# triq-org/spectroplot-js

Hardware: AMD Instinct MI355X
Metric: STFT frames/sec (N=1024 cf32) + IQ MSamples/s end-to-end to RGBA (higher is better)
Workload: dtype f64; 1 GPU; 16 MSample cf32, N=1024, Blackman-Harris, Viridis, gain 6, range 30, spectrogram layout, 16384 frames per GPU; format=CF32, n=1024, samples_per_gpu=16777216, frames_per_gpu=16384, window=blackmanHarris, cmap=viridis, generator=trinoise seed=0x5EED0001 step=7321 gshift=11 amp=0.5 namp=0.02

## Files before the change

### spectroplot-js_amd/binding.py

```python
import ctypes as C
import os
import weakref
import subprocess

import numpy as np

_HERE = os.path.dirname(os.path.abspath(__file__))

SP_CB_HIST_SIZE = 1000
FORMATS = ["CU4", "CS4", "CU8", "CS8", "CU12", "CS12", "CU16", "CS16", "CU32", "CS32", "CU64", "CS64", "CF32", "CF64"]

SP_ERR_NOT_POW2 = -2
SP_ERR_BYTE_LENGTH = -3
SP_ERR_UNSUPPORTED = -4
SP_ERR_NO_DEVICE = -5
SP_ERR_INVALID_ARG = -1

DETECTORS = {"sample": 0, "peak": 1}


def detector_id(detector):
    if detector not in DETECTORS:
        raise SpectroplotError(SP_ERR_INVALID_ARG, "detector must be 'sample' or 'peak', not %r" % (detector,))
    return DETECTORS[detector]
# ... 518 lines not shown

    def set_mean_window(self, nbytes=0):
        self._chk(self.lib.L.sp_context_set_mean_window(self.h, int(nbytes)))

    def render_index(self, fmt, data, n, windowc, block_norm, gain, rng, lut, width, channel_mode=False, waterfall=False,
                     detector="sample", want_index=True, fill=None):
        fid, _ = parse_format(fmt)
        data = np.ascontiguousarray(data, dtype=np.uint8)
        req, keep = _make_request(fid, n, windowc, block_norm, gain, rng, lut, channel_mode, waterfall, detector)
        W = int(width)
        L = len(keep[1])
        out, mm, rep = _host_reply(W, n, L, "index", 1, fill)
        self._chk(self.lib.L.sp_render_index(self.h, C.byref(req), _p(data), data.size, W, C.byref(rep),
                                             _p(out["index"]) if want_index else None))
        out["dBfs_min"], out["dBfs_max"] = float(mm[0]), float(mm[1])
        return out

    def index_to_rgba(self, d_index, pixels, lut, d_rgba):
        lut = np.ascontiguousarray(lut, dtype=np.uint8).reshape(-1, 3)
        self._chk(self.lib.L.sp_index_to_rgba(self.h, C.c_void_p(d_index or None), int(pixels), lut.ctypes.data_as(C.c_void_p), len(lut),
                                              C.c_void_p(d_rgba or None)))

    def render_density(self, fmt, data, n, windowc, block_norm, gain, rng, lut, width, channel_mode=False, waterfall=False,
                       detector="sample", fill=None):
        fid, _ = parse_format(fmt)
        data = np.ascontiguousarray(data, dtype=np.uint8)
        req, keep = _make_request(fid, n, windowc, block_norm, gain, rng, lut, channel_mode, waterfall, detector)
        out = np.full((int(n), len(keep[1])), 0 if fill is None else int(fill), np.uint32)
        self._chk(self.lib.L.sp_render_density(self.h, C.byref(req), data.ctypes.data_as(C.c_void_p), data.size, int(width),
                                               out.ctypes.data_as(C.c_void_p)))
        return out

    def density_from_index(self, d_index, n, width, waterfall, lut_len, d_density, accumulate=False):
        self._chk(self.lib.L.sp_density_from_index(self.h, C.c_void_p(d_index or None), int(n), int(width), int(bool(waterfall)),
                                                   int(lut_len), C.c_void_p(d_density or None), int(bool(accumulate))))

    def plan_creations(self):
        n = C.c_int64()
        self._chk(self.lib.L.sp_context_plan_creations(self.h, C.byref(n)))
        return n.value

    def plan(self, fmt, n, windowc, block_norm, gain, rng, lut, channel_mode=False, waterfall=False, detector="sample"):
        return Plan(self, fmt, n, windowc, block_norm, gain, rng, lut, channel_mode, waterfall, detector)


class Plan:

    def __init__(self, ctx, fmt, n, windowc, block_norm, gain, rng, lut, channel_mode=False, waterfall=False, detector="sample"):
        self.ctx = ctx
        self.detector = detector
        self.n = int(n)
        self.fid, self.sample_width = parse_format(fmt)
        req, keep = _make_request(self.fid, n, windowc, block_norm, gain, rng, lut, channel_mode, waterfall, detector)
        self.lut_len = len(keep[1])
        h = C.c_void_p()
        ctx._chk(ctx.lib.L.sp_plan_create(ctx.h, C.byref(req), C.byref(h)))
        self.h = h
        ctx._plans.add(self)

    def close(self):
        if self.h:
            self.ctx.lib.L.sp_plan_destroy(self.h)
            self.h = None

    def __del__(self):
        try:
            self.close()
        except Exception:
            pass

    def kernel_name(self, nbytes=None, width=None):
        if nbytes is None:
            return self.ctx.lib.L.sp_plan_kernel_name(self.h).decode()
        return self.ctx.lib.L.sp_plan_kernel_name_for(self.h, int(nbytes), int(width)).decode()

    def debug_launch(self, nbytes, width, rgba=0):
        out = np.zeros(len(LAUNCH_FIELDS), np.int64)
        used = C.c_size_t()
        self.ctx._chk(self.ctx.lib.L.sp_plan_debug_launch(self.h, int(nbytes), int(width), C.c_void_p(rgba or None),
                                                          out.ctypes.data_as(C.c_void_p), len(out), C.byref(used)))
        return _launch_dict(out)

    def force_kernel(self, which):
        self.ctx._chk(self.ctx.lib.L.sp_plan_force_kernel(self.h, {"auto": 0, "scratch": 1, "frames": 3}[which]))

    def execute(self, d_bytes, nbytes, width, rgba=0, gauge_mins=0, gauge_maxs=0, gauge_amps=0, c_hist=0, cb_hist=0, dbfs_minmax=0):
        rep = _device_reply(rgba, gauge_mins, gauge_maxs, gauge_amps, c_hist, cb_hist, dbfs_minmax)
        self.ctx._chk(self.ctx.lib.L.sp_plan_execute(self.h, C.c_void_p(d_bytes), nbytes, int(width), C.byref(rep)))

    def traces_kernel_name_for(self, nbytes, width):
        return self.ctx.lib.L.sp_plan_traces_kernel_name_for(self.h, int(nbytes), int(width)).decode()

    def execute_traces(self, d_bytes, nbytes, width, trace_min=0, trace_max=0):
        self.ctx._chk(self.ctx.lib.L.sp_plan_execute_traces(self.h, C.c_void_p(d_bytes or None), int(nbytes), int(width),
                                                            C.c_void_p(trace_min or None), C.c_void_p(trace_max or None)))

    def power_kernel_name_for(self, nbytes, width):
        return self.ctx.lib.L.sp_plan_power_kernel_name_for(self.h, int(nbytes), int(width)).decode()

    def execute_power(self, d_bytes, nbytes, width, d_power):
        self.ctx._chk(self.ctx.lib.L.sp_plan_execute_power(self.h, C.c_void_p(d_bytes or None), int(nbytes), int(width),
                                                           C.c_void_p(d_power or None)))

    def mean_kernel_name_for(self, nbytes, width):
        return self.ctx.lib.L.sp_plan_mean_kernel_name_for(self.h, int(nbytes), int(width)).decode()

    def execute_mean(self, d_bytes, nbytes, width, d_mean):
        self.ctx._chk(self.ctx.lib.L.sp_plan_execute_mean(self.h, C.c_void_p(d_bytes or None), int(nbytes), int(width),
                                                          C.c_void_p(d_mean or None)))

    def bandpower_kernel_name_for(self, nbytes, width):
        return self.ctx.lib.L.sp_plan_bandpower_kernel_name_for(self.h, int(nbytes), int(width)).decode()

    def execute_bandpower(self, d_bytes, nbytes, width, bands, d_band):
        b, count = _band_array(bands)
        self.ctx._chk(self.ctx.lib.L.sp_plan_execute_bandpower(self.h, C.c_void_p(d_bytes or None), int(nbytes), int(width),
                                                               _p(b) if count else None, count, C.c_void_p(d_band or None)))

    def power_to_db(self, d_power, count, d_db):
        self.ctx._chk(self.ctx.lib.L.sp_plan_power_to_db(self.h, C.c_void_p(d_power or None), int(count), C.c_void_p(d_db or None)))

    def index_kernel_name_for(self, nbytes, width):
        return self.ctx.lib.L.sp_plan_index_kernel_name_for(self.h, int(nbytes), int(width)).decode()

    def debug_index_launch(self, nbytes, width, index=0):
        out = np.zeros(len(LAUNCH_FIELDS), np.int64)
        used = C.c_size_t()
        self.ctx._chk(self.ctx.lib.L.sp_plan_debug_index_launch(self.h, int(nbytes), int(width), C.c_void_p(index or None),
                                                                out.ctypes.data_as(C.c_void_p), len(out), C.byref(used)))
        return _launch_dict(out)

    def execute_index(self, d_bytes, nbytes, width, index=0, rgba=0, gauge_mins=0, gauge_maxs=0, gauge_amps=0, c_hist=0, cb_hist=0,
                      dbfs_minmax=0):
        rep = _device_reply(rgba, gauge_mins, gauge_maxs, gauge_amps, c_hist, cb_hist, dbfs_minmax)
        self.ctx._chk(self.ctx.lib.L.sp_plan_execute_index(self.h, C.c_void_p(d_bytes or None), int(nbytes), int(width), C.byref(rep),
                                                           C.c_void_p(index or None)))

    def execute_density(self, d_bytes, nbytes, width, d_density, accumulate=False):
        self.ctx._chk(self.ctx.lib.L.sp_plan_execute_density(self.h, C.c_void_p(d_bytes or None), int(nbytes), int(width),
                                                             C.c_void_p(d_density or None), int(bool(accumulate))))

    def execute_batch(self, items):
        arr = (_BatchItem * max(len(items), 1))()
        keys = ("rgba", "gauge_mins", "gauge_maxs", "gauge_amps", "c_hist", "cb_hist", "dbfs_minmax")
        for k, (d_bytes, nbytes, width, outs) in enumerate(items):
            arr[k].bytes = d_bytes or None
            arr[k].nbytes = int(nbytes)
            arr[k].width = int(width)
            arr[k].reply = _device_reply(*[outs.get(key) for key in keys])
        self.ctx._chk(self.ctx.lib.L.sp_plan_execute_batch(self.h, arr, len(items)))

    def execute_from_host(self, data, width, rgba=0, gauge_mins=0, gauge_maxs=0, gauge_amps=0, c_hist=0, cb_hist=0, dbfs_minmax=0):
        data = np.ascontiguousarray(data, dtype=np.uint8)
        rep = _device_reply(rgba, gauge_mins, gauge_maxs, gauge_amps, c_hist, cb_hist, dbfs_minmax)
        self.ctx._chk(self.ctx.lib.L.sp_plan_execute_from_host(self.h, data.ctypes.data_as(C.c_void_p), data.size, int(width), C.byref(rep)))
        return data


class Group:

    def __init__(self, devices):
        self.lib = Library.get()
        arr = (C.c_int32 * len(devices))(*devices)
        h = C.c_void_p()
        self.lib.check(self.lib.L.sp_group_create(arr, len(devices), C.byref(h)))
        self.h = h
        self.size = len(devices)
# ... 52 lines not shown
```

### spectroplot-js_amd/csrc/sp_api.hip

```cpp
#include <hip/hip_runtime.h>

#include <cmath>
#include <cstdio>
#include <cstdlib>
#include <cstring>
#include <new>
#include <string>
#include <vector>

#include "../../include/spectroplot_hip.h"
#include "sp_geometry.h"
#include "sp_host.h"
#include "sp_kernel_frames_batch.h"
#include "sp_kernel_frames_peak.h"
#include "sp_kernel_frames_traces.h"
#include "sp_kernel_frames_power.h"
#include "sp_kernel_frames_index.h"
#include "sp_launch.h"
#include "sp_exact_sum.h"
#include "sp_cmap_tables.h"

namespace {

struct DeviceBuffer {
    void *p = nullptr;
    size_t cap = 0;
    int reserve(size_t bytes)
    {
        if (bytes <= cap) return SP_OK;
        if (p) (void)hipFree(p);
        p = nullptr;
        cap = 0;
        size_t want = bytes + bytes / 8 + 256;
        if (hipMalloc(&p, want) != hipSuccess) {
            if (hipMalloc(&p, bytes) != hipSuccess) return SP_ERR_NOMEM;
            want = bytes;
        }
        cap = want;
        return SP_OK;
    }
    void release()
    {
        if (p) (void)hipFree(p);
        p = nullptr;
        cap = 0;
    }
};

struct HostBuffer {
    void *p = nullptr;
    size_t cap = 0;
    int reserve(size_t bytes)
    {
        if (bytes <= cap) return SP_OK;
        if (p) (void)hipHostFree(p);
        p = nullptr;
        cap = 0;
        const size_t want = bytes + bytes / 8 + 256;
        if (hipHostMalloc(&p, want, hipHostMallocDefault) != hipSuccess) return SP_ERR_NOMEM;
        cap = want;
        return SP_OK;
    }
    void release()
    {
        if (p) (void)hipHostFree(p);
        p = nullptr;
        cap = 0;
    }
};

struct NamedRequest {
    std::string format, window, cmap;
    int32_t n = 0, channel_mode = 0, waterfall = 0;
    double gain = 0, range = 0;
    std::vector<double> windowc;
    std::vector<uint8_t> lut;
    double block_norm = 0;
    static std::string str(const char *s) { return s ? s : ""; }
    bool same(const sp_named_request &r) const
    {
        return !windowc.empty() && format == str(r.format) && window == str(r.window) && cmap == str(r.cmap) && n == r.n
               && channel_mode == (r.channel_mode ? 1 : 0) && waterfall == (r.waterfall ? 1 : 0) && !memcmp(&gain, &r.gain, 8)
               && !memcmp(&range, &r.range, 8);
    }
};

}

struct sp_context {
    int device = 0;
    hipStream_t own_stream = nullptr;
    hipStream_t stream = nullptr;
    std::string error;
    int cu_count = 256;
    DeviceBuffer frame_minmax;
    DeviceBuffer partial;
    DeviceBuffer scratch;
    DeviceBuffer traces_ws;
    DeviceBuffer power_plane;
    DeviceBuffer mean_ws;
    DeviceBuffer mean_window;
    size_t mean_window_bytes = 0;
    DeviceBuffer index_rgba;
    DeviceBuffer density_index;
    DeviceBuffer density_reply;
    DeviceBuffer in_bytes, out_rgba, render_small;
    HostBuffer host_small;
    hipStream_t copy_in = nullptr, copy_out = nullptr;
    hipEvent_t ev_arrived[spgeo::kMaxChunks] = {}, ev_rendered[spgeo::kMaxChunks] = {};
    sp_plan *cached_plan = nullptr;
    NamedRequest named;
    long long plans_created = 0;
    bool acc_dirty = false;
    size_t last_upload_bytes = 0;
    int last_chunks = 0;
    uint32_t seq = 0;
    DeviceBuffer batch_dev;
    HostBuffer batch_host;
    hipEvent_t ev_batch = nullptr;
    hipEvent_t ev_batch_done = nullptr;
    bool timing = false;
    hipEvent_t ev0 = nullptr, ev1 = nullptr;
    bool timed = false;
};

enum Kernel {
    kKernelAuto = 0,
    kKernelScratch = 1,
    kKernelLdsR16 = 2,
    kKernelFrames = 3,
    kKernelFramesPeak = 4,
};
static bool finishes_request(int kernel) { return kernel == kKernelFrames || kernel == kKernelFramesPeak; }

struct sp_plan {
    sp_context *ctx = nullptr;
    sp_request req{};
    std::vector<double> window;
    std::vector<uint8_t> lut;
    int levels = 0;
    spfmt::Format fmt{};
    double block_norm_db = 0;
    float gray_a = 0, gray_b = 0, cb_a = 0, cb_b = 0;
    bool edges_in_f32 = false;
    bool taper_finite = false;
    bool tw16_ok = false;
    sphost::Thresholds th{};
    DeviceBuffer tables;
    const double *d_window = nullptr, *d_cos = nullptr, *d_sin = nullptr, *d_gray_edge = nullptr, *d_cb_edge = nullptr;
    const uint32_t *d_lut = nullptr;
    const uint16_t *d_cell_g = nullptr, *d_cell_l = nullptr;
    const double2 *d_stage_tw = nullptr;
    DeviceBuffer ident_lut;
    int force_kernel = kKernelAuto;
};

namespace {

int fail(sp_context *ctx, int code, const std::string &msg)
{
    if (ctx) ctx->error = msg;
    return code;
}

int hip_fail(sp_context *ctx, hipError_t e, const char *what)
{
    return fail(ctx, SP_ERR_HIP, std::string(what) + ": " + hipGetErrorString(e));
}

#define SP_HIP(ctx, call)                                            \
    do {                                                             \
        hipError_t e_ = (call);                                      \
        if (e_ != hipSuccess) return hip_fail((ctx), e_, #call);     \
    } while (0)

int validate_request(sp_context *ctx, const sp_request *r)
{
    std::string why;
    const int rc = sphost::validate_request(r, why);
    return rc ? fail(ctx, rc, why) : SP_OK;
}

template <typename Body>
int timed(sp_context *ctx, Body &&body)
{
    if (ctx->timing) SP_HIP(ctx, hipEventRecord(ctx->ev0, ctx->stream));
    const int rc = body();
    if (rc) return rc;
    if (ctx->timing) {
        SP_HIP(ctx, hipEventRecord(ctx->ev1, ctx->stream));
        ctx->timed = true;
    }
    return SP_OK;
}

}


extern "C" int sp_version(void) { return SP_VERSION; }

extern "C" const char *sp_status_string(int status)
{
    switch (status) {
    case SP_OK: return "ok";
    case SP_ERR_INVALID_ARG: return "invalid argument";
    case SP_ERR_NOT_POW2: return "Length is not a power of 2";
    case SP_ERR_BYTE_LENGTH: return "byte length is not a multiple of the element size";
    case SP_ERR_UNSUPPORTED: return "unsupported by this library";
    case SP_ERR_NO_DEVICE: return "no HIP device";
    case SP_ERR_HIP: return "HIP runtime error";
    case SP_ERR_NOMEM: return "out of device memory";
    default: return "unknown status";
    }
}

extern "C" const char *sp_last_error(const sp_context *ctx) { return ctx ? ctx->error.c_str() : ""; }

extern "C" int sp_format_parse(const char *name, int32_t *format, int32_t *sample_width)
{
    const int32_t id = sphost::parse_format(name ? name : "");
    if (format) *format = id;
    if (sample_width) *sample_width = spfmt::describe(id).width;
    return SP_OK;
}

extern "C" int sp_format_element_size(int32_t format)
{
    if (format < 0 || format >= SP_FMT_COUNT) return SP_ERR_INVALID_ARG;
    return spfmt::describe(format).elem;
}

extern "C" int sp_slice_bounds(size_t nbytes, int32_t sample_width, int32_t index, int32_t count, size_t *begin, size_t *end)
{
    if (sample_width < 1 || count < 1 || index < 0 || index >= count || !begin || !end) return SP_ERR_INVALID_ARG;
    const size_t end_sample = nbytes / (size_t)sample_width;
// ... 243 lines not shown

extern "C" int sp_device_memset(sp_context *ctx, void *d_ptr, int value, size_t nbytes)
{
    if (!ctx) return SP_ERR_INVALID_ARG;
    SP_HIP(ctx, hipSetDevice(ctx->device));
    SP_HIP(ctx, hipMemsetAsync(d_ptr, value, nbytes, ctx->stream));
    return SP_OK;
}

extern "C" int sp_synth_trinoise(sp_context *ctx, void *d_bytes, int32_t format, uint64_t t0, uint64_t count, uint32_t seed,
                                 uint32_t step, uint32_t gshift, double amp, double namp)
{
    if (!ctx || !d_bytes) return SP_ERR_INVALID_ARG;
    if (format < 0 || format >= SP_FMT_COUNT) return fail(ctx, SP_ERR_INVALID_ARG, "unknown format id");
    if (count == 0) return SP_OK;
    SP_HIP(ctx, hipSetDevice(ctx->device));
    const spk::SynthArgs a{(uint8_t *)d_bytes, t0, count, seed, step, gshift, amp, namp};
    const int rc = spk::launch_synth_trinoise(a, format, ctx->stream);
    if (rc) return rc == SP_ERR_UNSUPPORTED ? fail(ctx, rc, "synth: too many samples for one launch") : rc;
    SP_HIP(ctx, hipGetLastError());
    return SP_OK;
}


extern "C" int sp_plan_create(sp_context *ctx, const sp_request *req, sp_plan **out)
{
    if (!ctx || !out) return SP_ERR_INVALID_ARG;
    *out = nullptr;
    int rc = validate_request(ctx, req);
    if (rc) return rc;
    SP_HIP(ctx, hipSetDevice(ctx->device));

    sp_plan *p = new (std::nothrow) sp_plan;
    if (!p) return fail(ctx, SP_ERR_NOMEM, "out of host memory");
    p->ctx = ctx;
    p->req = *req;
    p->window.assign(req->windowc, req->windowc + req->n);
    p->lut.assign(req->lut_rgb, req->lut_rgb + 3 * (size_t)req->lut_len);
    p->req.windowc = nullptr;
    p->req.lut_rgb = nullptr;
    p->levels = sphost::log2_exact(req->n);
    p->fmt = spfmt::describe(req->format);

    const int n = req->n, half = n / 2, L = req->lut_len;
    std::vector<double> ct((size_t)half), st((size_t)half);
    sphost::twiddles(n, ct.data(), st.data());
    const sphost::PixelMath pm(req->block_norm, req->gain, req->range, L);
    const sphost::Thresholds th = sphost::build_thresholds(pm, L);
    p->block_norm_db = pm.block_norm_db;
    p->gray_a = th.gray_a;
    p->gray_b = th.gray_b;
    p->cb_a = th.cb_a;
    p->cb_b = th.cb_b;
    p->edges_in_f32 = true;
    for (int g = 1; g < L; g++) p->edges_in_f32 &= th.gray_edge[(size_t)g] >= 0x1p-100 && th.gray_edge[(size_t)g] <= 0x1p100;
    for (int j = 1; j <= SP_CB_HIST_SIZE; j++) p->edges_in_f32 &= th.cb_edge[(size_t)j] >= 0x1p-100 && th.cb_edge[(size_t)j] <= 0x1p100;
    p->taper_finite = true;
    for (int i = 0; i < n; i++) p->taper_finite &= std::isfinite(p->window[(size_t)i]);
    p->tw16_ok = n >= 16;
    for (int k = 0; k < 8 && p->tw16_ok; k++)
        p->tw16_ok = ct[(size_t)k * (size_t)(n / 16)] == spk2::kTw16Host[k].c && st[(size_t)k * (size_t)(n / 16)] == spk2::kTw16Host[k].s;
    p->th = th;
    p->th.gray_edge.clear();
    p->th.cb_edge.clear();
    p->th.cell_g.clear();
    p->th.cell_l.clear();
    std::vector<uint32_t> lut32((size_t)L);
    for (int i = 0; i < L; i++)
        lut32[(size_t)i] = (uint32_t)p->lut[3 * (size_t)i] | ((uint32_t)p->lut[3 * (size_t)i + 1] << 8)
                           | ((uint32_t)p->lut[3 * (size_t)i + 2] << 16) | 0xff000000u;
    std::vector<double2> stage_tw;
    if (spk::frame_parts_support(n)) {
        stage_tw.resize((size_t)n);
        stage_tw[0] = make_double2(0, 0);
        for (int s = 1; s <= p->levels; s++) {
            const int cnt = 1 << (s - 1);
            for (int m = 0; m < cnt; m++) {
                const int k = m << (p->levels - s);
                stage_tw[(size_t)(cnt + m)] = make_double2(ct[(size_t)k], st[(size_t)k]);
            }
        }
    }

    const size_t nd = (size_t)n + 2 * (size_t)half + (size_t)L + (SP_CB_HIST_SIZE + 1) + 2 * stage_tw.size();
    const size_t cell_u16 = th.cell_g.size() + th.cell_l.size();
    const size_t bytes = nd * sizeof(double) + (((size_t)L * sizeof(uint32_t) + 7) & ~(size_t)7) + cell_u16 * sizeof(uint16_t);
    rc = p->tables.reserve(bytes);
    if (rc) {
        delete p;
        return fail(ctx, rc, "plan tables: out of device memory");
    }
    std::vector<uint8_t> host(bytes);
    double *h = (double *)host.data();
    double *d = (double *)p->tables.p;
    size_t o = 0;
    auto put = [&](const void *src, size_t count) {
        if (count) memcpy(h + o, src, count * sizeof(double));
        const double *dev = d + o;
        o += count;
        return dev;
    };
    p->d_window = put(p->window.data(), (size_t)n);
    p->d_cos = put(ct.data(), (size_t)half);
    p->d_sin = put(st.data(), (size_t)half);
    p->d_gray_edge = put(th.gray_edge.data(), (size_t)L);
    p->d_cb_edge = put(th.cb_edge.data(), SP_CB_HIST_SIZE + 1);
    p->d_stage_tw = (const double2 *)put(stage_tw.data(), 2 * stage_tw.size());
    memcpy(h + o, lut32.data(), (size_t)L * sizeof(uint32_t));
    p->d_lut = (const uint32_t *)(d + o);
    {
        const size_t off = o * sizeof(double) + (((size_t)L * sizeof(uint32_t) + 7) & ~(size_t)7);
        memcpy(host.data() + off, th.cell_g.data(), th.cell_g.size() * sizeof(uint16_t));
        memcpy(host.data() + off + th.cell_g.size() * sizeof(uint16_t), th.cell_l.data(), th.cell_l.size() * sizeof(uint16_t));
        p->d_cell_g = (const uint16_t *)((const char *)p->tables.p + off);
        p->d_cell_l = p->d_cell_g + th.cell_g.size();
    }
    hipError_t e = hipMemcpyAsync(p->tables.p, host.data(), bytes, hipMemcpyHostToDevice, ctx->stream);
    if (e == hipSuccess) e = hipStreamSynchronize(ctx->stream);
    if (e != hipSuccess) {
        p->tables.release();
        delete p;
        return hip_fail(ctx, e, "plan table upload");
    }
    ctx->plans_created++;
    *out = p;
    return SP_OK;
}

extern "C" int sp_context_plan_creations(const sp_context *ctx, int64_t *count)
{
    if (!ctx || !count) return SP_ERR_INVALID_ARG;
    *count = (int64_t)ctx->plans_created;
    return SP_OK;
}

extern "C" void sp_plan_destroy(sp_plan *plan)
{
    if (!plan) return;
    if (plan->ctx) {
        (void)hipSetDevice(plan->ctx->device);
        (void)hipStreamSynchronize(plan->ctx->stream);
        if (plan->ctx->cached_plan == plan) plan->ctx->cached_plan = nullptr;
    }
    plan->tables.release();
    plan->ident_lut.release();
    delete plan;
}

static bool plan_frames_capable(const sp_plan *plan)
{
    return spk2::frames_kernel_supports(plan->req.n) && plan->req.lut_len >= 2 && plan->req.lut_len <= spk::kLdsMaxLut
           && plan->gray_b <= spk::kLdsMaxGrayB && plan->edges_in_f32 && plan->taper_finite && plan->th.frames_ok && plan->tw16_ok;
}

static int plan_kernel(const sp_plan *plan)
{
    if (plan->force_kernel) return plan->force_kernel;
#ifdef SP_EXPERIMENT_KNOBS
    static const int env_kernel = getenv("SP_FORCE_KERNEL") ? atoi(getenv("SP_FORCE_KERNEL")) : 0;
    if (env_kernel == kKernelFrames && plan_frames_capable(plan)) return kKernelFrames;
    if (env_kernel == kKernelScratch) return kKernelScratch;
#endif
    return plan_frames_capable(plan) ? kKernelFrames : kKernelScratch;
}

static int request_kernel(const sp_plan *plan, int32_t peak_m)
{
    const int k = plan_kernel(plan);
    if (plan->req.detector != SP_DETECTOR_PEAK || peak_m < 2) return k;
    return k == kKernelFrames && spk2::frames_peak_supports(plan->req.n) ? kKernelFramesPeak : kKernelScratch;
}

extern "C" int sp_plan_force_kernel(sp_plan *plan, int32_t which)
{
    if (!plan || which < kKernelAuto || which > kKernelFrames) return SP_ERR_INVALID_ARG;
    if (which == kKernelLdsR16) return fail(plan->ctx, SP_ERR_UNSUPPORTED, "k_lds_r16 is no longer part of the library");
    if (which == kKernelFrames && !plan_frames_capable(plan)) return fail(plan->ctx, SP_ERR_UNSUPPORTED, "k_frames does not cover this request");
    plan->force_kernel = which;
    return SP_OK;
}

static const char *kernel_name(int kernel)
{
    return kernel == kKernelFramesPeak ? "frames_peak" : kernel == kKernelFrames ? "frames" : "scratch_radix2";
}

extern "C" const char *sp_plan_kernel_name(const sp_plan *plan) { return plan ? kernel_name(request_kernel(plan, 2)) : ""; }

extern "C" const char *sp_plan_kernel_name_for(const sp_plan *plan, size_t nbytes, int32_t width)
{
    return plan ? kernel_name(request_kernel(plan, spgeo::peak_shape(spgeo::geometry(plan->fmt, plan->req.n, nbytes, width)).m)) : "";
}

struct PackedSource {
    const void *bytes;
    size_t nbytes;
    double stride;
};

static void plan_frame_args(const sp_plan *plan, spk::FrameArgs &a)
{
    a.n = plan->req.n;
    a.levels = plan->levels;
    a.channel_mode = plan->req.channel_mode ? 1 : 0;
    a.waterfall = plan->req.waterfall ? 1 : 0;
    a.lut_len = plan->req.lut_len;
    a.sample_width = plan->fmt.width;
    a.window = plan->d_window;
    a.cos_t = plan->d_cos;
    a.sin_t = plan->d_sin;
    a.gray_edge = plan->d_gray_edge;
    a.cb_edge = plan->d_cb_edge;
    a.lut_rgba = plan->d_lut;
    a.gray_a = plan->gray_a;
    a.gray_b = plan->gray_b;
    a.cb_a = plan->cb_a;
    a.cb_b = plan->cb_b;
    a.g2_a = plan->th.g2_a;
    a.g2_b = plan->th.g2_b;
    a.g2_thr = plan->th.g2_thr;
    a.g2_m = plan->th.g2_m;
    a.c2_a = plan->th.c2_a;
    a.c2_b = plan->th.c2_b;
    a.c2_thr = plan->th.c2_thr;
    a.c2_m = plan->th.c2_m;
    a.c2_lo = plan->th.c2_lo;
    a.c2_hi = plan->th.c2_hi;
    a.block_norm_db = plan->block_norm_db;
    a.gain = plan->req.gain;
    a.range = plan->req.range;
    a.cell_g = plan->d_cell_g;
    a.cell_l = plan->d_cell_l;
    a.cells = plan->th.cells;
}

struct RequestShape {
    spgeo::Geometry g;
    spgeo::PeakShape peak;
};

static RequestShape request_shape(const sp_plan *plan, size_t nbytes, int32_t width)
{
    const spgeo::Geometry g = spgeo::geometry(plan->fmt, plan->req.n, nbytes, width);
    return {g, plan->req.detector == SP_DETECTOR_PEAK ? spgeo::peak_shape(g) : spgeo::PeakShape{}};
}

static int check_capture(sp_context *ctx, const spfmt::Format &f, int n, const void *bytes, size_t nbytes, int32_t width, const sp_reply *reply,
                         const std::string &who)
{
    const bool item = !who.empty();
    if (width < 0) return fail(ctx, SP_ERR_INVALID_ARG, who + "width < 0");
    if (nbytes && !bytes) return fail(ctx, SP_ERR_INVALID_ARG, who + (item ? "bytes is null" : "d_bytes is null"));
    if (nbytes % (size_t)f.elem) return fail(ctx, SP_ERR_BYTE_LENGTH, who + "byte length is not a multiple of the element size");
    if ((double)nbytes / (double)f.width >= 2147483648.0 - (double)n)
        return fail(ctx, SP_ERR_UNSUPPORTED, who + "captures of 2^31 samples or more must be sliced (sample positions are int32)");
    if ((double)width * (double)n > 4e12) return fail(ctx, SP_ERR_UNSUPPORTED, who + "image too large");
    if (reply && (((uintptr_t)reply->c_hist | (uintptr_t)reply->cb_hist | (uintptr_t)reply->dbfs_minmax) & 7) != 0)
        return fail(ctx, SP_ERR_INVALID_ARG, (item ? who : "reply: ") + "c_hist, cb_hist and dbfs_minmax must be 8-byte aligned");
    return SP_OK;
}
// ... 84 lines not shown
struct Picture {
    enum Kind { kRgba, kIndexFrames, kIndexExtract } kind;
    uint8_t *image;
};

static Picture index_picture(uint8_t *d_index, bool frames)
{
    return Picture{frames ? Picture::kIndexFrames : d_index ? Picture::kIndexExtract : Picture::kRgba, d_index};
}

static int plan_execute_range(sp_plan *plan, const void *d_bytes, const RequestShape &shape, int32_t x_begin, int32_t x_end, bool first,
                              bool last, const sp_reply *out, const Picture &pic, const PackedSource *src = nullptr)
{
    if (!plan || !out) return SP_ERR_INVALID_ARG;
    sp_context *ctx = plan->ctx;
    const spgeo::Geometry &g = shape.g;
    const spgeo::PeakShape &peak = shape.peak;
    const int n = plan->req.n;
    const int32_t width = g.width;
    int rc = device_operands(ctx, plan->fmt, n, d_bytes, g.nbytes, width, out, "sp_plan_execute");
    if (rc) return rc;
    hipStream_t s = ctx->stream;

    if (width == 0) {
        if (out->c_hist) SP_HIP(ctx, hipMemsetAsync(out->c_hist, 0, (size_t)plan->req.lut_len * sizeof(uint64_t), s));
        if (out->cb_hist) SP_HIP(ctx, hipMemsetAsync(out->cb_hist, 0, SP_CB_HIST_SIZE * sizeof(uint64_t), s));
        if (out->dbfs_minmax) {
            static const double init[2] = {0.0, -200.0};
            SP_HIP(ctx, hipMemcpyAsync(out->dbfs_minmax, init, sizeof init, hipMemcpyHostToDevice, s));
            SP_HIP(ctx, hipStreamSynchronize(s));
        }
        return SP_OK;
    }

    const int which = request_kernel(plan, peak.m);
    if (src && which != kKernelFrames) return fail(ctx, SP_ERR_INVALID_ARG, "a packed source is for the frame-loop kernel only");
    rc = finishes_request(which) ? SP_OK : ctx->frame_minmax.reserve(2 * (size_t)width * sizeof(double));
    if (rc) return fail(ctx, rc, "workspace: out of device memory");
    const size_t acc_bytes = 64 + (SP_MAX_LUT + SP_CB_HIST_SIZE) * sizeof(unsigned long long);
    const bool fresh_partial = ctx->partial.cap < acc_bytes;
    rc = ctx->partial.reserve(acc_bytes);
    if (rc) return fail(ctx, rc, "workspace: out of device memory");
    if (first && (fresh_partial || ctx->acc_dirty)) {
        static const unsigned long long mm_init[2] = {0x7ff0000000000000ull, 0ull};
        SP_HIP(ctx, hipMemsetAsync(ctx->partial.p, 0, ctx->partial.cap, s));
        SP_HIP(ctx, hipMemcpyAsync((char *)ctx->partial.p + 16, mm_init, sizeof mm_init, hipMemcpyHostToDevice, s));
        SP_HIP(ctx, hipStreamSynchronize(s));
    }
    ctx->acc_dirty = true;

    spk::FrameArgs a{};
    plan_frame_args(plan, a);
    frame_source_args(a, plan, d_bytes, g, x_begin, x_end, src);
    a.frame_min = (double *)ctx->frame_minmax.p;
    a.frame_max = a.frame_min + width;
    a.scratch = nullptr;
    if (first && ++ctx->seq == 0) ctx->seq = 1;
    a.first = first ? 1 : 0;
    a.seq = ctx->seq;
    a.flag = (unsigned int *)ctx->partial.p;
    a.gauge_mins = out->gauge_mins;
    a.gauge_maxs = out->gauge_maxs;
    a.gauge_amps = out->gauge_amps;
    a.out_c = (unsigned long long *)out->c_hist;
    a.out_cb = (unsigned long long *)out->cb_hist;
    a.out_minmax = out->dbfs_minmax;

    a.mm_acc = (unsigned long long *)((char *)ctx->partial.p + 16);
    a.c_hist = (unsigned long long *)((char *)ctx->partial.p + 64);
    a.cb_hist = a.c_hist + SP_MAX_LUT;
    const bool extract = pic.kind == Picture::kIndexExtract;
    a.rgba = extract ? (uint8_t *)ctx->index_rgba.p : pic.image;
    a.rgba_fast = pic.kind == Picture::kIndexFrames ? index_fast(a.rgba, width, n, x_begin, x_end) : rgba_fast(a.rgba, width, n);
    if (extract) a.lut_rgba = (const uint32_t *)plan->ident_lut.p;

    const int32_t peak_nsamp = (int32_t)(peak.nsamp < 2147483647 ? peak.nsamp : 2147483647);
    rc = timed(ctx, [&]() -> int {
        int r = SP_OK;
        if (pic.kind == Picture::kIndexFrames) {
            if (which != kKernelFrames) return fail(ctx, SP_ERR_INVALID_ARG, "k_frames_index renders what k_frames renders");
            r = spk2::launch_frames_index(a, plan->req.format, plan->d_stage_tw, ctx->cu_count, ctx->device, s);
            if (r) return fail(ctx, r, "k_frames_index launch rejected the configuration");
        } else if (which == kKernelFrames) {
            r = spk2::launch_frames(a, plan->req.format, plan->d_stage_tw, ctx->cu_count, ctx->device, s);
            if (r) return fail(ctx, r, "k_frames launch rejected the configuration");
        } else if (which == kKernelFramesPeak) {
            r = spk2::launch_frames_peak(a, plan->req.format, plan->d_stage_tw, peak.m, peak_nsamp, ctx->cu_count, ctx->device, s);
            if (r) return fail(ctx, r, "k_frames_peak launch rejected the configuration");
        } else {
            const bool hold = peak.m >= 2;
            unsigned blocks;
            r = scratch_reserve(ctx, a, hold ? 3 : 2, x_end - x_begin, &blocks);
            if (r) return r;
            r = spk::launch_scratch_radix2(a, plan->req.format, blocks, hold, peak.m, peak_nsamp, s);
            if (r) return fail(ctx, r, "bad format");
        }
        SP_HIP(ctx, hipGetLastError());
        if (extract && x_end > x_begin) return extract_index_band(ctx, a.rgba, pic.image, width, n, plan->req.waterfall != 0, x_begin, x_end);
        return SP_OK;
    });
    if (rc) return rc;

    if (!last) return SP_OK;
    if (finishes_request(which)) {
        ctx->acc_dirty = false;
        return SP_OK;
    }

    spk::FinishArgs fa{};
    fa.bytes = a.bytes;
    fa.nbytes = a.nbytes;
    fa.nelem = a.nelem;
    fa.stride = a.stride;
    fa.n = n;
    fa.width = width;
    fa.format = plan->req.format;
    fa.block_norm_db = plan->block_norm_db;
    fa.gain = plan->req.gain;
    fa.range = plan->req.range;
    fa.frame_min = a.frame_min;
    fa.frame_max = a.frame_max;
    fa.gauge_mins = out->gauge_mins;
    fa.gauge_maxs = out->gauge_maxs;
    fa.gauge_amps = out->gauge_amps;
    fa.mm_acc = a.mm_acc;
    fa.out_minmax = out->dbfs_minmax;
    fa.lut_len = plan->req.lut_len;
    fa.acc_c = a.c_hist;
    fa.acc_cb = a.cb_hist;
    fa.out_c = (unsigned long long *)out->c_hist;
    fa.out_cb = (unsigned long long *)out->cb_hist;
    spk::launch_finish_frames(fa, s);
    SP_HIP(ctx, hipGetLastError());
    ctx->acc_dirty = false;
    return SP_OK;
}

extern "C" int sp_plan_execute(sp_plan *plan, const void *d_bytes, size_t nbytes, int32_t width, const sp_reply *out)
{
    if (!plan || !out) return SP_ERR_INVALID_ARG;
    return plan_execute_range(plan, d_bytes, request_shape(plan, nbytes, width), 0, width < 0 ? 0 : width, true, true, out,
                              Picture{Picture::kRgba, out->rgba});
}

extern "C" int sp_plan_debug_launch(const sp_plan *plan, size_t nbytes, int32_t width, const void *rgba, int64_t *out, size_t capacity,
                                    size_t *used)
{
    if (!plan || !plan->ctx || width < 0 || !used) return SP_ERR_INVALID_ARG;
    const RequestShape shape = request_shape(plan, nbytes, width);
    const spgeo::Geometry &g = shape.g;
    const int n = plan->req.n, cu_count = plan->ctx->cu_count;
    const int which = width == 0 ? kKernelAuto : request_kernel(plan, shape.peak.m);
    spk2::FramesLaunch fl{0, 0, 0, 0};
    int prefetch = 0;
    if (finishes_request(which)) {
        prefetch = spk2::frames_prefetch_width(plan->fmt.width, g.in_bounds, g.stride, g.width);
        if (spk2::frames_launch_rule(n, plan->req.lut_len, width, cu_count, 0, fl)) return SP_ERR_UNSUPPORTED;
    }
    const int64_t v[] = {which, plan->levels, plan->req.channel_mode ? 1 : 0, prefetch, fl.gf, fl.groups, fl.grid, fl.lds_bytes,
                         rgba_fast((const uint8_t *)rgba, width, n) ? 1 : 0, shape.peak.m, cu_count};
    *used = sizeof v / sizeof v[0];
    if (*used > capacity || !out) return SP_ERR_INVALID_ARG;
    memcpy(out, v, sizeof v);
    return SP_OK;
}

extern "C" int sp_debug_frames_launch(int32_t n, int32_t lut_len, int64_t count, int32_t cu_count, int32_t gf_fixed, int64_t *out,
// ... 1379 lines not shown
```

### spectroplot-js_amd/csrc/sp_frames_table_loads.inc.h

```cpp
        constexpr int WINK = WIN_LDS ? (N + kThreads - 1) / kThreads : 1;
        double win_r[WINK];
        if constexpr (WIN_LDS) {
#pragma unroll
            for (int k = 0; k < WINK; k++) {
                const int i = tid + k * kThreads, e = i / T, t = i % T;
                win_r[k] = i < N ? a.window[rev4(e) * T + (int)(__brev((unsigned)t) >> (32 - (LOG2N - 4)))] : 0.0;
            }
        }
        constexpr int NTW = frames_tw_entries(N);
        constexpr int TWK = (NTW + kThreads - 1) / kThreads;
        double2 tw_r[TWK > 0 ? TWK : 1];
#pragma unroll
        for (int k = 0; k < TWK; k++) {
            const int i = tid + k * kThreads;
            tw_r[k] = i < NTW ? stage_tw[i] : make_double2(0.0, 0.0);
        }
        const unsigned int lut_r = tid < a.lut_len ? a.lut_rgba[tid] : 0u;
        double cb_r[(SP_CB_HIST_SIZE + kThreads) / kThreads];
        const double ge_r = tid < a.lut_len ? a.gray_edge[tid] : 0.0;
#pragma unroll
        for (int k = 0; k < (SP_CB_HIST_SIZE + kThreads) / kThreads; k++) {
            const int i = tid + k * kThreads;
            cb_r[k] = i <= SP_CB_HIST_SIZE ? a.cb_edge[i] : 0.0;
        }
```

### spectroplot-js_amd/csrc/sp_frames_table_stores.inc.h

```cpp
        for (int i = tid; i < a.cells; i += kThreads) s_cells[i] = 0;
        if (tid < 8) s_done[tid] = 0;
        if (tid < 2) s_red[tid] = tid ? -200.0 : 0.0;
        for (int i = tid; i < (LATE_SIDE ? 2 : 1) * group_frames * MMS; i += kThreads) {
            s_mm[2 * i] = 0x7ff0000000000000ull;
            s_mm[2 * i + 1] = 0ull;
        }
#pragma unroll
        for (int k = 0; k < TWK; k++) {
            const int i = tid + k * kThreads;
            if (i < NTW) s_tw[i] = tw_r[k];
        }
        if (tid < a.lut_len) s_lut[tid] = lut_r;
        if (tid < a.lut_len) ((double *)(smem + lay.off_gedge))[tid] = ge_r;
#pragma unroll
        for (int k = 0; k < (SP_CB_HIST_SIZE + kThreads) / kThreads; k++) {
            const int i = tid + k * kThreads;
            if (i <= SP_CB_HIST_SIZE) ((double *)(smem + lay.off_cbedge))[i] = cb_r[k];
        }
        if constexpr (WIN_LDS) {
#pragma unroll
            for (int k = 0; k < WINK; k++) {
                const int i = tid + k * kThreads;
                if (i < N) s_win[i] = win_r[k];
            }
        }
```

### spectroplot-js_amd/csrc/sp_host.cpp

```cpp
#include "sp_host.h"

#include <cctype>
#include <cmath>
#include <cstring>

namespace sphost {

int32_t parse_format(const char *name)
{
    char f[24];
    size_t i = 0;
    for (; name && name[i] && i + 1 < sizeof f; i++) f[i] = (char)toupper((unsigned char)name[i]);
    f[i] = 0;
    static const struct { const char *name; int32_t id; } table[] = {
        {"CU4", SP_FMT_CU4}, {"CS4", SP_FMT_CS4}, {"CU8", SP_FMT_CU8}, {"DATA", SP_FMT_CU8}, {"COMPLEX16U", SP_FMT_CU8},
        {"CS8", SP_FMT_CS8}, {"COMPLEX16S", SP_FMT_CS8}, {"CU16", SP_FMT_CU16}, {"CS16", SP_FMT_CS16},
        {"CU12", SP_FMT_CU12}, {"CS12", SP_FMT_CS12}, {"CU32", SP_FMT_CU32}, {"CS32", SP_FMT_CS32},
        {"CU64", SP_FMT_CU64}, {"CS64", SP_FMT_CS64}, {"CF32", SP_FMT_CF32}, {"CFILE", SP_FMT_CF32},
        {"COMPLEX", SP_FMT_CF32}, {"CF64", SP_FMT_CF64},
    };
    for (const auto &e : table)
        if (!strcmp(f, e.name)) return e.id;
    return SP_FMT_CU8;
}
// ... 259 lines not shown
        auto count_le = [](const std::vector<double> &edge, double v) {
            int32_t lo = 0, hi = (int32_t)edge.size() - 1;
            while (lo < hi) {
                const int32_t mid = (lo + hi + 1) >> 1;
                if (edge[(size_t)mid] <= v) lo = mid;
                else hi = mid - 1;
            }
            return lo;
        };
        t.cells = end + 2;
        t.cell_g.assign((size_t)lut_len + 1, (uint16_t)end);
        t.cell_l.assign(SP_CB_HIST_SIZE + 2, (uint16_t)end);
        t.cell_g[0] = 0;
        t.cell_l[0] = 0;
        for (int32_t g = 1; g < lut_len; g++)
            if (t.gray_edge[(size_t)g] != spjs::inf()) t.cell_g[(size_t)g] = (uint16_t)(g + count_le(t.cb_edge, t.gray_edge[(size_t)g]));
        for (int32_t l = 1; l <= SP_CB_HIST_SIZE; l++)
            if (t.cb_edge[(size_t)l] != spjs::inf()) t.cell_l[(size_t)l] = (uint16_t)(l + count_le(t.gray_edge, t.cb_edge[(size_t)l]));
    }
    auto fractf_ = [](float v) { return v - std::floor(v); };
    t.frames_ok = g_m < 0.125 && c_m < 0.125 && l_max < 120.0 && std::isfinite(t.g2_a) && std::isfinite(t.c2_a) && fractf_(t.c2_lo) >= t.c2_thr
                  && fractf_(t.c2_hi) >= t.c2_thr && t.c2_hi < (float)SP_CB_HIST_SIZE;
    return t;
}

sp_reply ReplyRecord::view(void *base) const
{
    sp_reply r{};
    r.c_hist = (uint64_t *)base;
    r.cb_hist = r.c_hist + lut_len;
    r.dbfs_minmax = (double *)(r.cb_hist + SP_CB_HIST_SIZE);
    r.gauge_mins = (uint8_t *)(r.dbfs_minmax + 2);
    r.gauge_maxs = r.gauge_mins + width;
    r.gauge_amps = r.gauge_maxs + width;
    return r;
}

void ReplyRecord::unpack_side(const void *base, const sp_reply &to) const
{
    const sp_reply h = view(const_cast<void *>(base));
    if (to.c_hist) memcpy(to.c_hist, h.c_hist, lut_len * 8);
    if (to.cb_hist) memcpy(to.cb_hist, h.cb_hist, SP_CB_HIST_SIZE * 8);
    if (to.dbfs_minmax) memcpy(to.dbfs_minmax, h.dbfs_minmax, 16);
}

void ReplyRecord::unpack_gauges(const void *base, const sp_reply &to, size_t at) const
{
    const sp_reply h = view(const_cast<void *>(base));
    if (to.gauge_mins) memcpy(to.gauge_mins + at, h.gauge_mins, width);
    if (to.gauge_maxs) memcpy(to.gauge_maxs + at, h.gauge_maxs, width);
    if (to.gauge_amps) memcpy(to.gauge_amps + at, h.gauge_amps, width);
}

int validate_request(const sp_request *r, std::string &why)
{
    const auto no = [&](int code, const char *msg) {
        why = msg;
        return code;
    };
    if (!r) return no(SP_ERR_INVALID_ARG, "request is null");
    if (r->format < 0 || r->format >= SP_FMT_COUNT) return no(SP_ERR_INVALID_ARG, "unknown format id");
    if (r->n < 1 || log2_exact(r->n) < 0) return no(SP_ERR_NOT_POW2, "Length is not a power of 2");
    if (r->n < 2) return no(SP_ERR_UNSUPPORTED, "n = 1 is not supported (the reference writes no pixels for it)");
    if (r->n > SP_MAX_N) return no(SP_ERR_UNSUPPORTED, "n exceeds SP_MAX_N");
    if (r->lut_len < 1 || r->lut_len > SP_MAX_LUT) return no(SP_ERR_UNSUPPORTED, "lut_len must be 1..SP_MAX_LUT");
    if (!r->windowc || !r->lut_rgb) return no(SP_ERR_INVALID_ARG, "windowc / lut_rgb is null");
    if (!(r->range > 0) || !std::isfinite(r->range)) return no(SP_ERR_UNSUPPORTED, "range must be finite and > 0");
    if (!std::isfinite(r->gain)) return no(SP_ERR_UNSUPPORTED, "gain must be finite");
    if (r->detector != SP_DETECTOR_SAMPLE && r->detector != SP_DETECTOR_PEAK)
        return no(SP_ERR_INVALID_ARG, "detector must be SP_DETECTOR_SAMPLE or SP_DETECTOR_PEAK");
    return SP_OK;
}

bool same_request(const sp_request &q, const std::vector<double> &window, const std::vector<uint8_t> &lut, const sp_request *r)
{
    if (q.format != r->format || q.n != r->n || q.channel_mode != r->channel_mode || q.waterfall != r->waterfall || q.lut_len != r->lut_len
        || q.detector != r->detector)
        return false;
    if (memcmp(&q.block_norm, &r->block_norm, 8) || memcmp(&q.gain, &r->gain, 8) || memcmp(&q.range, &r->range, 8)) return false;
    if (window.size() != (size_t)r->n || memcmp(window.data(), r->windowc, sizeof(double) * (size_t)r->n)) return false;
    return lut.size() == 3 * (size_t)r->lut_len && memcmp(lut.data(), r->lut_rgb, lut.size()) == 0;
}

}
```

### spectroplot-js_amd/csrc/sp_host.h

```cpp
#pragma once

#include <cstdint>
#include <string>
#include <vector>

#include "../../include/spectroplot_hip.h"
#include "sp_formats.h"

namespace sphost {

int32_t parse_format(const char *name);

int32_t log2_exact(int64_t n);

void twiddles(int32_t n, double *cos_table, double *sin_table);

bool window(const char *name, int32_t n, double *out, double *weight);

int32_t lookup_key(const char *const *keys, int32_t count, const char *name);
const char *window_by_name(const char *name);

bool cmap_generate(const char *key, int32_t stops, uint8_t *rgb);

struct PixelMath {
    double block_norm_db;
    double gain, range;
    double color_max;
    double color_norm;

    PixelMath(double block_norm, double gain, double range, int32_t lut_len);
    double dbfs(double abs2) const;
    double rel_db(double abs2) const;
    int32_t gray(double abs2) const;
    int32_t centibel(double abs2) const;
};

struct Thresholds {
    std::vector<double> gray_edge;
    std::vector<double> cb_edge;
    float gray_a, gray_b, cb_a, cb_b;
    float g2_a, g2_b, g2_thr, g2_m;
    float c2_a, c2_b, c2_thr, c2_m, c2_lo, c2_hi;
    bool frames_ok;
    std::vector<uint16_t> cell_g;
    std::vector<uint16_t> cell_l;
    int32_t cells;
};
Thresholds build_thresholds(const PixelMath &pm, int32_t lut_len);

struct ReplyRecord {
    size_t lut_len, width;
    size_t words() const { return lut_len + SP_CB_HIST_SIZE + 2; }
    size_t bytes() const { return words() * 8 + 3 * width; }
    sp_reply view(void *base) const;
    void unpack_side(const void *base, const sp_reply &to) const;
    void unpack_gauges(const void *base, const sp_reply &to, size_t at = 0) const;
};

int validate_request(const sp_request *r, std::string &why);

bool same_request(const sp_request &kept, const std::vector<double> &window, const std::vector<uint8_t> &lut, const sp_request *r);

}
```

### spectroplot-js_amd/csrc/sp_inst_frames.hip

```cpp
#include "sp_kernel_frames_batch.h"
#include "sp_kernel_frames_index.h"
#include "sp_kernel_frames_peak.h"
#include "sp_kernel_frames_power.h"
#include "sp_kernel_frames_traces.h"
```

Before: 250.0 million frames/s.

## Preload kernel prologue tables from a single packed device image

Result: no change. 251.5 million frames/s, median of 6 (+0.6%).

```diff
diff --git a/spectroplot-js_amd/binding.py b/spectroplot-js_amd/binding.py
--- a/spectroplot-js_amd/binding.py
+++ b/spectroplot-js_amd/binding.py
@@ -624,7 +624,7 @@
         return _launch_dict(out)
 
     def force_kernel(self, which):
-        self.ctx._chk(self.ctx.lib.L.sp_plan_force_kernel(self.h, {"auto": 0, "scratch": 1, "frames": 3}[which]))
+        self.ctx._chk(self.ctx.lib.L.sp_plan_force_kernel(self.h, {"auto": 0, "scratch": 1, "frames": 3, "frames_pinned": 5}[which]))
 
     def execute(self, d_bytes, nbytes, width, rgba=0, gauge_mins=0, gauge_maxs=0, gauge_amps=0, c_hist=0, cb_hist=0, dbfs_minmax=0):
         rep = _device_reply(rgba, gauge_mins, gauge_maxs, gauge_amps, c_hist, cb_hist, dbfs_minmax)
diff --git a/spectroplot-js_amd/csrc/sp_api.hip b/spectroplot-js_amd/csrc/sp_api.hip
--- a/spectroplot-js_amd/csrc/sp_api.hip
+++ b/spectroplot-js_amd/csrc/sp_api.hip
@@ -16,6 +16,7 @@
 #include "sp_kernel_frames_traces.h"
 #include "sp_kernel_frames_power.h"
 #include "sp_kernel_frames_index.h"
+#include "sp_kernel_frames_trim.h"
 #include "sp_launch.h"
 #include "sp_exact_sum.h"
 #include "sp_cmap_tables.h"
@@ -130,6 +131,7 @@
     kKernelLdsR16 = 2,
     kKernelFrames = 3,
     kKernelFramesPeak = 4,
+    kKernelFramesPinned = 5,
 };
 static bool finishes_request(int kernel) { return kernel == kKernelFrames || kernel == kKernelFramesPeak; }
 
@@ -151,6 +153,7 @@
     const uint32_t *d_lut = nullptr;
     const uint16_t *d_cell_g = nullptr, *d_cell_l = nullptr;
     const double2 *d_stage_tw = nullptr;
+    const uint4 *d_table_image = nullptr;
     DeviceBuffer ident_lut;
     int force_kernel = kKernelAuto;
 };
@@ -560,9 +563,14 @@
         }
     }
 
+    std::vector<uint8_t> image;
+    if (spk2::frames_trim_supports(n) && L >= 2 && L <= spk::kLdsMaxLut)
+        image = sphost::table_image(n, L, spk::kLdsMaxLut, spk2::frames_tw_entries(n), spk::lds_win_in_lds(n), lut32.data(),
+                                    (const double *)stage_tw.data(), th.gray_edge.data(), th.cb_edge.data(), p->window.data());
     const size_t nd = (size_t)n + 2 * (size_t)half + (size_t)L + (SP_CB_HIST_SIZE + 1) + 2 * stage_tw.size();
     const size_t cell_u16 = th.cell_g.size() + th.cell_l.size();
-    const size_t bytes = nd * sizeof(double) + (((size_t)L * sizeof(uint32_t) + 7) & ~(size_t)7) + cell_u16 * sizeof(uint16_t);
+    const size_t image_off = (nd * sizeof(double) + (((size_t)L * sizeof(uint32_t) + 7) & ~(size_t)7) + cell_u16 * sizeof(uint16_t) + 15) & ~(size_t)15;
+    const size_t bytes = image_off + image.size();
     rc = p->tables.reserve(bytes);
     if (rc) {
         delete p;
@@ -593,6 +601,10 @@
         p->d_cell_g = (const uint16_t *)((const char *)p->tables.p + off);
         p->d_cell_l = p->d_cell_g + th.cell_g.size();
     }
+    if (!image.empty()) {
+        memcpy(host.data() + image_off, image.data(), image.size());
+        p->d_table_image = (const uint4 *)((const char *)p->tables.p + image_off);
+    }
     hipError_t e = hipMemcpyAsync(p->tables.p, host.data(), bytes, hipMemcpyHostToDevice, ctx->stream);
     if (e == hipSuccess) e = hipStreamSynchronize(ctx->stream);
     if (e != hipSuccess) {
@@ -633,7 +645,7 @@
 
 static int plan_kernel(const sp_plan *plan)
 {
-    if (plan->force_kernel) return plan->force_kernel;
+    if (plan->force_kernel) return plan->force_kernel == kKernelFramesPinned ? kKernelFrames : plan->force_kernel;
 #ifdef SP_EXPERIMENT_KNOBS
     static const int env_kernel = getenv("SP_FORCE_KERNEL") ? atoi(getenv("SP_FORCE_KERNEL")) : 0;
     if (env_kernel == kKernelFrames && plan_frames_capable(plan)) return kKernelFrames;
@@ -651,9 +663,9 @@
 
 extern "C" int sp_plan_force_kernel(sp_plan *plan, int32_t which)
 {
-    if (!plan || which < kKernelAuto || which > kKernelFrames) return SP_ERR_INVALID_ARG;
+    if (!plan || which < kKernelAuto || which == kKernelFramesPeak || which > kKernelFramesPinned) return SP_ERR_INVALID_ARG;
     if (which == kKernelLdsR16) return fail(plan->ctx, SP_ERR_UNSUPPORTED, "k_lds_r16 is no longer part of the library");
-    if (which == kKernelFrames && !plan_frames_capable(plan)) return fail(plan->ctx, SP_ERR_UNSUPPORTED, "k_frames does not cover this request");
+    if ((which == kKernelFrames || which == kKernelFramesPinned) && !plan_frames_capable(plan)) return fail(plan->ctx, SP_ERR_UNSUPPORTED, "k_frames does not cover this request");
     plan->force_kernel = which;
     return SP_OK;
 }
@@ -904,7 +916,9 @@
             r = spk2::launch_frames_index(a, plan->req.format, plan->d_stage_tw, ctx->cu_count, ctx->device, s);
             if (r) return fail(ctx, r, "k_frames_index launch rejected the configuration");
         } else if (which == kKernelFrames) {
-            r = spk2::launch_frames(a, plan->req.format, plan->d_stage_tw, ctx->cu_count, ctx->device, s);
+            if (plan->d_table_image && spk2::frames_trim_chosen(a) && plan->force_kernel != kKernelFramesPinned && !extract)
+                r = spk2::launch_frames_trim(a, plan->req.format, plan->d_table_image, ctx->cu_count, ctx->device, s);
+            else r = spk2::launch_frames(a, plan->req.format, plan->d_stage_tw, ctx->cu_count, ctx->device, s);
             if (r) return fail(ctx, r, "k_frames launch rejected the configuration");
         } else if (which == kKernelFramesPeak) {
             r = spk2::launch_frames_peak(a, plan->req.format, plan->d_stage_tw, peak.m, peak_nsamp, ctx->cu_count, ctx->device, s);
diff --git a/spectroplot-js_amd/csrc/sp_frames_table_image_loads.inc.h b/spectroplot-js_amd/csrc/sp_frames_table_image_loads.inc.h
--- /dev/null
+++ b/spectroplot-js_amd/csrc/sp_frames_table_image_loads.inc.h
@@ -0,0 +1,10 @@
+        constexpr int NTW = frames_tw_entries(N);
+        constexpr int IMGK = (spimg::spans(kLdsMaxLut, NTW, kLdsMaxLut, WIN_LDS ? N : 0).total / 16 + kThreads - 1) / kThreads;
+        const spimg::Spans img = spimg::spans(kLdsMaxLut, NTW, a.lut_len, WIN_LDS ? N : 0);
+        uint4 img_r[IMGK];
+#pragma unroll
+        for (int k = 0; k < IMGK; k++) {
+            const int i = tid + k * kThreads;
+            img_r[k] = i * 16 < img.total ? (SP_TABLE_IMAGE)[i] : make_uint4(0u, 0u, 0u, 0u);
+        }
+        asm volatile("s_barrier" ::: "memory");
diff --git a/spectroplot-js_amd/csrc/sp_frames_table_image_stores.inc.h b/spectroplot-js_amd/csrc/sp_frames_table_image_stores.inc.h
--- /dev/null
+++ b/spectroplot-js_amd/csrc/sp_frames_table_image_stores.inc.h
@@ -0,0 +1,7 @@
+        (void)s_lut;
+#pragma unroll
+        for (int k = 0; k < IMGK; k++) {
+            const int b = (tid + k * kThreads) * 16;
+            const int at = b < img.tw ? kOffLut + b : b < img.win ? lay.off_tw + (b - img.tw) : lay.off_win + (b - img.win);
+            if (b < img.total) *(uint4 *)(smem + at) = img_r[k];
+        }
diff --git a/spectroplot-js_amd/csrc/sp_frames_table_loads.inc.h b/spectroplot-js_amd/csrc/sp_frames_table_loads.inc.h
--- a/spectroplot-js_amd/csrc/sp_frames_table_loads.inc.h
+++ b/spectroplot-js_amd/csrc/sp_frames_table_loads.inc.h
@@ -1,3 +1,6 @@
+#ifdef SP_TABLE_IMAGE
+#include "sp_frames_table_image_loads.inc.h"
+#else
         constexpr int WINK = WIN_LDS ? (N + kThreads - 1) / kThreads : 1;
         double win_r[WINK];
         if constexpr (WIN_LDS) {
@@ -23,3 +26,4 @@
             const int i = tid + k * kThreads;
             cb_r[k] = i <= SP_CB_HIST_SIZE ? a.cb_edge[i] : 0.0;
         }
+#endif
diff --git a/spectroplot-js_amd/csrc/sp_frames_table_stores.inc.h b/spectroplot-js_amd/csrc/sp_frames_table_stores.inc.h
--- a/spectroplot-js_amd/csrc/sp_frames_table_stores.inc.h
+++ b/spectroplot-js_amd/csrc/sp_frames_table_stores.inc.h
@@ -5,6 +5,9 @@
             s_mm[2 * i] = 0x7ff0000000000000ull;
             s_mm[2 * i + 1] = 0ull;
         }
+#ifdef SP_TABLE_IMAGE
+#include "sp_frames_table_image_stores.inc.h"
+#else
 #pragma unroll
         for (int k = 0; k < TWK; k++) {
             const int i = tid + k * kThreads;
@@ -24,3 +27,4 @@
                 if (i < N) s_win[i] = win_r[k];
             }
         }
+#endif
diff --git a/spectroplot-js_amd/csrc/sp_host.cpp b/spectroplot-js_amd/csrc/sp_host.cpp
--- a/spectroplot-js_amd/csrc/sp_host.cpp
+++ b/spectroplot-js_amd/csrc/sp_host.cpp
@@ -365,4 +365,30 @@
     return lut.size() == 3 * (size_t)r->lut_len && memcmp(lut.data(), r->lut_rgb, lut.size()) == 0;
 }
 
-}
+static_assert(spimg::kCbEdges == SP_CB_HIST_SIZE + 1, "the table image holds every centi-bel edge");
+
+std::vector<uint8_t> table_image(int32_t n, int32_t lut_len, int32_t lut_slots, int32_t tw_entries, bool win_in_lds, const uint32_t *lut_rgba,
+                                 const double *stage_tw, const double *gray_edge, const double *cb_edge, const double *window)
+{
+    const spimg::Spans sp = spimg::spans(lut_slots, tw_entries, lut_len, win_in_lds ? n : 0);
+    std::vector<uint8_t> img((size_t)sp.total, 0);
+    if (lut_len > lut_slots || n < 16 || log2_exact(n) < 0) return img;
+    memcpy(img.data(), lut_rgba, (size_t)lut_len * 4);
+    memcpy(img.data() + sp.tw, stage_tw, (size_t)tw_entries * 16);
+    memcpy(img.data() + sp.gedge, gray_edge, (size_t)lut_len * 8);
+    memcpy(img.data() + sp.cbedge, cb_edge, (size_t)spimg::kCbEdges * 8);
+    if (win_in_lds) {
+        const int32_t T = n / 16, bits = log2_exact(n) - 4;
+        for (int32_t e = 0; e < 16; e++) {
+            const int32_t re = ((e & 1) << 3) | ((e & 2) << 1) | ((e & 4) >> 1) | ((e & 8) >> 3);
+            for (int32_t t = 0; t < T; t++) {
+                int32_t rt = 0;
+                for (int32_t b = 0; b < bits; b++) rt |= ((t >> b) & 1) << (bits - 1 - b);
+                memcpy(img.data() + sp.win + (size_t)(e * T + t) * 8, window + re * T + rt, 8);
+            }
+        }
+    }
+    return img;
+}
+
+}
diff --git a/spectroplot-js_amd/csrc/sp_host.h b/spectroplot-js_amd/csrc/sp_host.h
--- a/spectroplot-js_amd/csrc/sp_host.h
+++ b/spectroplot-js_amd/csrc/sp_host.h
@@ -6,6 +6,7 @@
 
 #include "../../include/spectroplot_hip.h"
 #include "sp_formats.h"
+#include "sp_table_image.h"
 
 namespace sphost {
 
@@ -61,4 +62,7 @@
 
 bool same_request(const sp_request &kept, const std::vector<double> &window, const std::vector<uint8_t> &lut, const sp_request *r);
 
+std::vector<uint8_t> table_image(int32_t n, int32_t lut_len, int32_t lut_slots, int32_t tw_entries, bool win_in_lds, const uint32_t *lut_rgba,
+                                 const double *stage_tw, const double *gray_edge, const double *cb_edge, const double *window);
+
 }
diff --git a/spectroplot-js_amd/csrc/sp_inst_frames.hip b/spectroplot-js_amd/csrc/sp_inst_frames.hip
--- a/spectroplot-js_amd/csrc/sp_inst_frames.hip
+++ b/spectroplot-js_amd/csrc/sp_inst_frames.hip
@@ -3,3 +3,4 @@
 #include "sp_kernel_frames_peak.h"
 #include "sp_kernel_frames_power.h"
 #include "sp_kernel_frames_traces.h"
+#include "sp_kernel_frames_trim.h"
diff --git a/spectroplot-js_amd/csrc/sp_kernel_frames_trim.h b/spectroplot-js_amd/csrc/sp_kernel_frames_trim.h
--- /dev/null
+++ b/spectroplot-js_amd/csrc/sp_kernel_frames_trim.h
@@ -0,0 +1,60 @@
+#pragma once
+
+#include "sp_kernel_frames.h"
+#include "sp_table_image.h"
+
+namespace spk2 {
+
+constexpr int kTrimMaxLog2N = 10;
+
+constexpr bool frames_trim_variant_built(int n, bool ch, int prefetch)
+{
+    return !ch && ((n == 1024 && prefetch == 8) || (n == 512 && prefetch == 2));
+}
+__host__ __device__ inline bool frames_trim_supports(int n) { return n == 512 || n == 1024; }
+
+inline size_t frames_trim_image_bytes(int n, int lut_len)
+{
+    return (size_t)spimg::spans(kLdsMaxLut, frames_tw_entries(n), lut_len, lds_win_in_lds(n) ? n : 0).total;
+}
+
+template <int LOG2N, bool CH, int PFB>
+__global__ __launch_bounds__(kFrameThreads, 1) void k_frames_trim(const FrameArgs a, const int format, const double2 *__restrict__ stage_tw,
+                                                            const int group_frames, const int groups)
+{
+    static_assert(LOG2N <= kTrimMaxLog2N && frames_tw_entries(1 << LOG2N) == (1 << LOG2N) && frames_tw_max_stage(1 << LOG2N) >= LOG2N,
+                  "every table of the prologue is in the image, every twiddle in LDS");
+#define SP_TABLE_IMAGE ((const uint4 *)stage_tw)
+#include "sp_frames_request_body.inc.h"
+#undef SP_TABLE_IMAGE
+}
+
+#define SP_SIZES_9_10(X, ...) X(9, __VA_ARGS__) X(10, __VA_ARGS__)
+SP_DECLARE_LAUNCH_N(launch_frames_trim_n, SP_SIZES_9_10)
+
+#ifdef SP_INST_TRIM_LOG2N
+template <>
+int launch_frames_trim_n<SP_INST_TRIM_LOG2N>(SP_LAUNCH_N_PARAMS)
+{
+    constexpr int L = SP_INST_TRIM_LOG2N;
+    SP_LAUNCH_VARIANT_IF(frames_trim_variant_built, k_frames_trim)
+}
+#endif
+
+inline bool frames_trim_chosen(const FrameArgs &a)
+{
+    return frames_trim_supports(a.n)
+           && frames_trim_variant_built(a.n, a.channel_mode != 0, frames_prefetch_width(a.sample_width, a.in_bounds, a.stride, a.width));
+}
+
+inline int launch_frames_trim(const FrameArgs &a, int format, const uint4 *table_image, int cu_count, int device, hipStream_t stream)
+{
+    const double2 *const stage_tw = (const double2 *)table_image;
+    const int prefetch = frames_prefetch_width(a.sample_width, a.in_bounds, a.stride, a.width);
+    FramesLaunch fl;
+    if (!frames_trim_supports(a.n) || !table_image || frames_launch_rule(a.n, a.lut_len, a.x_end - a.frame0, cu_count, 0, fl))
+        return SP_ERR_UNSUPPORTED;
+    SP_LAUNCH_LEVELS(SP_SIZES_9_10, launch_frames_trim_n)
+}
+
+}
diff --git a/spectroplot-js_amd/csrc/sp_table_image.h b/spectroplot-js_amd/csrc/sp_table_image.h
--- /dev/null
+++ b/spectroplot-js_amd/csrc/sp_table_image.h
@@ -0,0 +1,28 @@
+#pragma once
+
+#ifdef __HIPCC__
+#define SP_IMG_HD __host__ __device__
+#else
+#define SP_IMG_HD
+#endif
+
+namespace spimg {
+
+constexpr int kCbEdges = 1001;
+
+struct Spans {
+    int tw, gedge, cbedge, win, total;
+};
+
+SP_IMG_HD inline constexpr Spans spans(int lut_slots, int tw_entries, int lut_len, int win_entries)
+{
+    Spans s{};
+    s.tw = lut_slots * 4;
+    s.gedge = s.tw + tw_entries * 16;
+    s.cbedge = s.gedge + lut_len * 8;
+    s.win = (s.cbedge + kCbEdges * 8 + 15) & ~15;
+    s.total = (s.win + win_entries * 8 + 15) & ~15;
+    return s;
+}
+
+}
```
